# KMASAHIRO/AVR

Measured on AMD Instinct MI355X. Metric: ray-samples/sec/GPU (1024 rays×256 samp×512 freq) + IR render ms/pose, higher is better.
Workload: dtype f32; 1 GPU; c2_meshrir_1024x256x512; mode=pose, rays=1024, samples=256, T=1022, freq_bins=512, distinct_poses=16, parallelism=poses x1 (no data-path collective)

## Files before the change

avr_amd/csrc/render_fwd.hip:

```cpp
#include "common.h"

#include <cstdlib>

using namespace avr;

typedef float floatx16 __attribute__((ext_vector_type(16)));

namespace {

constexpr double kTwoPi = 6.283185307179586476925286766559;

__global__ void tables_kernel(avr_render_params p, float* __restrict__ d_vals,
                              float* __restrict__ frac, int32_t* __restrict__ shift,
                              float* __restrict__ pl, float2* __restrict__ phase,
                              float2* __restrict__ tw) {
    const int S = p.n_samples, T = p.T, F = T / 2 + 1;
    const int64_t gid = (int64_t)blockIdx.x * blockDim.x + threadIdx.x;
    const int64_t stride = (int64_t)gridDim.x * blockDim.x;
    for (int64_t i = gid; i < S; i += stride) {
        const float d = linspace_at(0.0f, 1.0f, S, (int)i) * p.depth_scale + p.depth_offset;
        const float fr = (p.fs * d) / p.speed;
        d_vals[i] = d;
        frac[i] = fr;
        shift[i] = (int32_t)rintf(fr);
// ... 232 lines not shown
            const float al = alpha[s];
            alpha[s] = trans * al;
            trans = trans * ((1.0f - al) + 1e-6f);
        }
    }
    __syncthreads();
    if (active)
        for (int s = lane; s < S; s += 64) w_out[base + s] = alpha[s];
}

constexpr int kMaxReduceThreads = 1024;
constexpr int kMaxGroupRays = 4096;

template <typename Tin, bool VECTOR, int CPT, int kUnroll, int G, int MAXT>
__global__ __launch_bounds__(MAXT) void ray_reduce_fwd_kernel(
    avr_render_params pp, const Tin* __restrict__ sig, const float* __restrict__ w,
    const int32_t* __restrict__ delay, float* __restrict__ part, int B, int R, int S, int T,
    int rays_per_split, int64_t total) {
    constexpr int VEC = VECTOR ? Vec16<Tin>::N : 1;
    extern __shared__ float lds_wd[];
    const int nthreads = blockDim.x;
    const int split = blockIdx.x, s0 = blockIdx.y * G, b = blockIdx.z;
    const int gcount = min(G, S - s0);
    const int r0 = split * rays_per_split;
    const int nr = max(0, min(R, r0 + rays_per_split) - r0);
    float* w_l = lds_wd;
    int* d_l = reinterpret_cast<int*>(lds_wd + G * max(nr, 1));
    for (int i = threadIdx.x; i < G * nr; i += nthreads) {
        const int g = i / nr, rr = i - g * nr;
        if (g < gcount) {
            const int64_t idx = ((int64_t)b * R + r0 + rr) * S + s0 + g;
            w_l[i] = w[idx];
            d_l[i] = delay[idx];
        } else {
            w_l[i] = 0.0f;
            d_l[i] = 0x7fffffff;
        }
    }
    __syncthreads();
    const int64_t row0 = (((int64_t)b * R + r0) * S + s0) * (int64_t)T;
    const int L = gcount * T;
    const int phase = (int)(row0 % VEC);
    const int nchunks = (L + phase + VEC - 1) / VEC;
    const int64_t row_stride = (int64_t)S * T;

    float acc[CPT][VEC];
    int tk[CPT][VEC];
    int tm[CPT][VEC];
    int gk[CPT][VEC];
    int tmax[CPT][G];
    int lim[G];
#pragma unroll
    for (int g = 0; g < G; ++g) lim[g] = tail_limit(pp, min(s0 + g, S - 1));
#pragma unroll
    for (int c = 0; c < CPT; ++c) {
#pragma unroll
        for (int g = 0; g < G; ++g) tmax[c][g] = -1;
#pragma unroll
        for (int k = 0; k < VEC; ++k) {
            acc[c][k] = 0.0f;
            const int e = (threadIdx.x + c * nthreads) * VEC + k - phase;
            const bool ok = e >= 0 && e < L;
            const int g = (G == 1) ? 0 : (ok ? e / T : 0);
            gk[c][k] = g;
            tk[c][k] = ok ? e - g * T : -1;
            int l = lim[0];
#pragma unroll
            for (int q = 1; q < G; ++q)
                if (g == q) l = lim[q];
            tm[c][k] = (tk[c][k] >= 0 && tk[c][k] < l) ? tk[c][k] : -1;
#pragma unroll
            for (int q = 0; q < G; ++q)
                if (g == q) tmax[c][q] = max(tmax[c][q], tm[c][k]);
        }
    }

    auto live = [&](int r, int c) {
        bool any = false;
#pragma unroll
        for (int g = 0; g < G; ++g) any |= tmax[c][g] >= d_l[g * nr + r];
        return any;
    };
    auto load_chunk = [&](int64_t rowbase, int c, bool need, float* x) {
        const int j = threadIdx.x + c * nthreads;
        if constexpr (VECTOR) {
            load16_masked(sig + rowbase, (uint32_t)nchunks * 16u,
                          need ? (uint32_t)j * 16u : kSkip, x);
        } else {
            const int64_t e0 = rowbase + j;
            x[0] = (need && j < nchunks && e0 < total) ? load_f(sig, e0) : 0.0f;
        }
    };
    auto accumulate = [&](int r, float (*x)[VEC]) {
        float wg[G];
        int dg[G];
#pragma unroll
        for (int g = 0; g < G; ++g) {
            wg[g] = w_l[g * nr + r];
            dg[g] = d_l[g * nr + r];
        }
#pragma unroll
        for (int c = 0; c < CPT; ++c)
#pragma unroll
            for (int k = 0; k < VEC; ++k) {
                float ws = wg[0];
                int ds = dg[0];
#pragma unroll
                for (int g = 1; g < G; ++g)
                    if (gk[c][k] == g) {
                        ws = wg[g];
                        ds = dg[g];
                    }
                const float wm = (tm[c][k] >= ds) ? ws : 0.0f;
                acc[c][k] = fmaf(wm, x[c][k], acc[c][k]);
            }
    };

    int r = 0;
    for (; r + kUnroll <= nr; r += kUnroll) {
        float x[kUnroll][CPT][VEC];
        bool need[kUnroll][CPT];
#pragma unroll
        for (int u = 0; u < kUnroll; ++u)
#pragma unroll
            for (int c = 0; c < CPT; ++c) need[u][c] = live(r + u, c);
#pragma unroll
        for (int u = 0; u < kUnroll; ++u) {
            const int64_t rowbase = row0 + (int64_t)(r + u) * row_stride - phase;
#pragma unroll
            for (int c = 0; c < CPT; ++c) load_chunk(rowbase, c, need[u][c], x[u][c]);
        }
#pragma unroll
        for (int u = 0; u < kUnroll; ++u) accumulate(r + u, x[u]);
    }
    for (; r < nr; ++r) {
        const int64_t rowbase = row0 + (int64_t)r * row_stride - phase;
        float x[CPT][VEC];
#pragma unroll
        for (int c = 0; c < CPT; ++c) load_chunk(rowbase, c, live(r, c), x[c]);
        accumulate(r, x);
    }
#pragma unroll
    for (int c = 0; c < CPT; ++c)
#pragma unroll
        for (int k = 0; k < VEC; ++k) {
            const int t = tk[c][k];
            if (t >= 0) part[(((int64_t)split * B + b) * S + s0 + gk[c][k]) * T + t] = acc[c][k];
        }
}

constexpr int kDftThreads = 256;
constexpr int kKc = 64;

template <int NS>
__global__ __launch_bounds__(kDftThreads) void dft_phase_fwd_kernel(
    avr_render_params pp, const float* __restrict__ part, const float* __restrict__ pl,
    const int32_t* __restrict__ shift, const float2* __restrict__ phase,
    const float2* __restrict__ twg, float2* __restrict__ spart, int B, int S, int T, int KS,
    int kchunk, int xcd_order) {
    extern __shared__ float2 tw[];
    __shared__ float As[32][kKc + 1];
    const int F = T / 2 + 1;
    const int P = ((S + 31) / 32) * KS;
    (void)P;
    const int nfb = (F + 127) / 128, nst = (S + 31) / 32;
    const int per = KS * nfb;
    int stile, q;
    if (xcd_order) {
        const int L = blockIdx.x, xcd = L & 7;
        q = L >> 3;
        stile = (q / per) * 8 + xcd;
        if (stile >= nst) return;
    } else {
        stile = blockIdx.x / per;
        q = blockIdx.x;
    }
    const int ks = (q % per) / nfb, fblk = (q % per) % nfb;
    const int b = blockIdx.z;
    const int wave = threadIdx.x >> 6, lane = threadIdx.x & 63;
    const int fbase = fblk * 128 + wave * 32;
    const int f = fbase + (lane & 31);
    const int fm = (f < F) ? f : 0;
    const int half = lane >> 5;
    const int col = threadIdx.x & 63, row0 = threadIdx.x >> 6;
    int sh[8];
    bool srow[8];
#pragma unroll
    for (int i = 0; i < 8; ++i) {
        const int s = stile * 32 + row0 + 4 * i;
        srow[i] = s < S;
        sh[i] = receiver_shift(pp, min(s, S - 1));
    }
    (void)shift;
    const int64_t slab = (int64_t)B * S * T;
    const int s_first = min(stile * 32 + row0, S - 1);
    const int64_t rowbase0 = ((int64_t)b * S + s_first) * T;
    const int64_t max_row_off = ((int64_t)b * S + (S - 1)) * T;

    const int k0 = ks * kchunk;
    const int k1 = min(T, k0 + kchunk);
    floatx16 acc_re, acc_im;
#pragma unroll
    for (int i = 0; i < 16; ++i) {
        acc_re[i] = 0.0f;
        acc_im[i] = 0.0f;
    }
    const int inc = (int)((2LL * fm) % T);
    float raw[NS][8], g[8];
    auto issue = [&](int kc) {
        const int tc = min(kc + col, T - 1);
#pragma unroll
        for (int k = 0; k < NS; ++k)
#pragma unroll
            for (int i = 0; i < 8; ++i) {
                const int64_t ro = min(rowbase0 + (int64_t)(4 * i) * T, max_row_off);
                raw[k][i] = part[k * slab + ro + tc];
            }
#pragma unroll
        for (int i = 0; i < 8; ++i) g[i] = pl[sh[i] + tc];
    };
    auto commit = [&](int kc) {
        const int t = kc + col;
#pragma unroll
        for (int i = 0; i < 8; ++i) {
            float sum = raw[0][i];
#pragma unroll
            for (int k = 1; k < NS; ++k) sum += raw[k][i];
            const bool ok = srow[i] && t < k1 && t < T - 1 - sh[i];
            As[row0 + 4 * i][col] = ok ? sum * g[i] : 0.0f;
        }
    };
    if (k0 < k1) issue(k0);
    stage_table<kDftThreads>(tw, twg, T);
    for (int kc = k0; kc < k1; kc += kKc) {
        __syncthreads();
        commit(kc);
        __syncthreads();
        if (kc + kKc < k1) issue(kc + kKc);
        int idx = (int)(((int64_t)(kc + half) * fm) % T);
#pragma unroll 8
        for (int kk = 0; kk < kKc; kk += 2) {
            const float a = As[lane & 31][kk + half];
            float2 c = tw[idx];
            asm volatile("" : "+v"(c.x), "+v"(c.y));
            acc_re = __builtin_amdgcn_mfma_f32_32x32x2f32(a, c.x, acc_re, 0, 0, 0);
            acc_im = __builtin_amdgcn_mfma_f32_32x32x2f32(a, c.y, acc_im, 0, 0, 0);
            idx += inc;
            if (idx >= T) idx -= T;
        }
    }
    float re = 0.0f, im = 0.0f;
    {
        float2 ph[16];
#pragma unroll
        for (int reg = 0; reg < 16; ++reg) {
            const int s = stile * 32 + (reg & 3) + 8 * (reg >> 2) + 4 * half;
            ph[reg] = phase[(int64_t)min(s, S - 1) * F + fm];
        }
#pragma unroll
        for (int reg = 0; reg < 16; ++reg) asm volatile("" ::"v"(ph[reg].x), "v"(ph[reg].y));
#pragma unroll
        for (int reg = 0; reg < 16; ++reg) {
            const int s = stile * 32 + (reg & 3) + 8 * (reg >> 2) + 4 * half;
            if (s < S) {
                const float zr = acc_re[reg], zi = acc_im[reg];
                re += zr * ph[reg].x - zi * ph[reg].y;
                im += zr * ph[reg].y + zi * ph[reg].x;
            }
        }
    }
    re += __shfl_xor(re, 32, 64);
    im += __shfl_xor(im, 32, 64);
    if (half == 0 && f < F) {
        spart[((int64_t)b * P + stile * KS + ks) * F + f] = make_float2(re, im);
    }
}

__global__ __launch_bounds__(256) void spectrum_finalize_kernel(int B, int P, int F,
                                                                const float2* __restrict__ spart,
                                                                float2* __restrict__ out) {
    __shared__ float2 red[16][17];
    const int b = blockIdx.y;
    const int g = threadIdx.x >> 4, j = threadIdx.x & 15;
    const int f = blockIdx.x * 16 + j;
    const int fc = min(f, F - 1);
    const float2* src = spart + (int64_t)b * P * F + fc;
    float ax = 0.f, ay = 0.f;
    for (int q0 = 0; q0 < P; q0 += 64) {
        float2 v[4];
#pragma unroll
        for (int u = 0; u < 4; ++u) v[u] = src[(int64_t)min(q0 + g + 16 * u, P - 1) * F];
#pragma unroll
        for (int u = 0; u < 4; ++u)
            if (q0 + g + 16 * u < P) {
                ax += v[u].x;
                ay += v[u].y;
            }
    }
    red[g][j] = make_float2(ax, ay);
    __syncthreads();
    if (g == 0 && f < F) {
        float2 r = red[0][j];
        for (int k = 1; k < 16; ++k) {
            r.x += red[k][j].x;
            r.y += red[k][j].y;
        }
        out[(int64_t)b * F + f] = r;
    }
}

__global__ __launch_bounds__(256) void irfft_kernel(int F, int B1, const float2* __restrict__ spec,
                                                    const float2* __restrict__ spec2,
                                                    const float2* __restrict__ twg,
                                                    float* __restrict__ ir, float* __restrict__ ir2) {
    extern __shared__ float2 lds[];
    __shared__ float red[8][33];
    const int n = 2 * (F - 1);
    float2* X = lds;
    float2* tw = lds + F;
    int b = blockIdx.y;
    if (b >= B1) {
        b -= B1;
        spec = spec2;
        ir = ir2;
    }
    stage_table<256>(X, spec + (int64_t)b * F, F);
    stage_table<256>(tw, twg, n);
    __syncthreads();
    const int tl = threadIdx.x & 31, slice = threadIdx.x >> 5;
    const int t = blockIdx.x * 32 + tl;
    const int tm = (t < n) ? t : 0;
    float acc[4] = {0.f, 0.f, 0.f, 0.f};
    int idx[4];
#pragma unroll
    for (int c = 0; c < 4; ++c) idx[c] = (int)(((int64_t)(1 + slice + 8 * c) * tm) % n);
    const int step4 = (int)((32LL * tm) % n);
    int k = 1 + slice;
    for (; k + 24 < F - 1; k += 32) {
#pragma unroll
        for (int c = 0; c < 4; ++c) {
            const float2 w = tw[idx[c]];
            const float2 x = X[k + 8 * c];
            acc[c] += x.x * w.x - x.y * w.y;
            idx[c] += step4;
            if (idx[c] >= n) idx[c] -= n;
        }
    }
    for (; k < F - 1; k += 8) {
        const int id = (int)(((int64_t)k * tm) % n);
        const float2 w = tw[id];
        const float2 x = X[k];
        acc[0] += x.x * w.x - x.y * w.y;
    }
    red[slice][tl] = (acc[0] + acc[1]) + (acc[2] + acc[3]);
    __syncthreads();
    if (slice == 0 && t < n) {
        float s = 0.0f;
#pragma unroll
        for (int q = 0; q < 8; ++q) s += red[q][tl];
        const float nyq = (t & 1) ? -X[F - 1].x : X[F - 1].x;
        const float v = (X[0].x + nyq) + 2.0f * s;
        ir[(int64_t)b * n + t] = v / (float)n;
    }
}

__global__ __launch_bounds__(256) void irfft_bwd_kernel(int F, const float* __restrict__ gir,
                                                        const float2* __restrict__ twg,
                                                        float2* __restrict__ grad) {
    extern __shared__ float lds_irb[];
    __shared__ float2 red[8][33];
    const int n = 2 * (F - 1);
    const int b = blockIdx.y;
    float2* tw = reinterpret_cast<float2*>(lds_irb);
    float* g = lds_irb + 2 * n;
    stage_table<256>(tw, twg, n);
    for (int i = threadIdx.x; i < n; i += 256) g[i] = gir[(int64_t)b * n + i];
    __syncthreads();
    const int kl = threadIdx.x & 31, sl = threadIdx.x >> 5;
    const int k = blockIdx.x * 32 + kl;
    const int km = k < F ? k : 0;
    int idx = (int)(((int64_t)km * sl) % n);
    const int step = (int)(((int64_t)km * 8) % n);
    float ac = 0.f, as = 0.f;
    for (int t = sl; t < n; t += 8) {
        const float2 c = tw[idx];
        ac = fmaf(g[t], c.x, ac);
        as = fmaf(g[t], c.y, as);
        idx += step;
        if (idx >= n) idx -= n;
    }
    red[sl][kl] = make_float2(ac, as);
    __syncthreads();
    if (sl == 0 && k < F) {
        float2 r = red[0][kl];
        for (int q = 1; q < 8; ++q) {
            r.x += red[q][kl].x;
            r.y += red[q][kl].y;
        }
        const bool edge = (k == 0) || (k == F - 1);
// ... 153 lines not shown
        (void)hipFuncSetAttribute((const void*)weights_fwd_kernel<__hip_bfloat16>,
                                  hipFuncAttributeMaxDynamicSharedMemorySize, (int)lds);
    }
    if (attn_dtype == AVR_DTYPE_F32)
        hipLaunchKernelGGL(weights_fwd_kernel<float>, grid, dim3(256), lds, as_stream(stream), *p,
                           (int)B, (const float*)attn, rays_o, pos_tx, dirs, d_vals, w, delay);
    else if (attn_dtype == AVR_DTYPE_F16)
        hipLaunchKernelGGL(weights_fwd_kernel<__half>, grid, dim3(256), lds, as_stream(stream),
                           *p, (int)B, (const __half*)attn, rays_o, pos_tx, dirs, d_vals, w, delay);
    else if (attn_dtype == AVR_DTYPE_BF16)
        hipLaunchKernelGGL(weights_fwd_kernel<__hip_bfloat16>, grid, dim3(256), lds,
                           as_stream(stream), *p, (int)B, (const __hip_bfloat16*)attn, rays_o,
                           pos_tx, dirs, d_vals, w, delay);
    else
        return fail(AVR_E_ARG, "avr_weights_fwd: unknown attn dtype");
    return check_launch("avr_weights_fwd");
}


namespace {
int reduce_variant() { return 2; }

struct ReduceShape {
    int G, cpt, threads;
};

template <int VEC>
ReduceShape reduce_shape(int S, int T) {
    ReduceShape sh;
    sh.G = 1;
    int max_phase = 0;
    for (int s0 = 0; s0 < S && s0 < VEC * sh.G; s0 += sh.G)
        max_phase = max(max_phase, (int)(((int64_t)s0 * T) % VEC));
    const int nch = (sh.G * T + max_phase + VEC - 1) / VEC;
    sh.cpt = 1;
    while ((nch + sh.cpt - 1) / sh.cpt > kMaxReduceThreads) ++sh.cpt;
    const int need = (nch + sh.cpt - 1) / sh.cpt;
    sh.threads = max(64, (need + 63) / 64 * 64);
    return sh;
}

template <typename Tin, bool VECTOR, int C, int G>
void launch_reduce_v(dim3 grid, dim3 block, size_t lds, hipStream_t st, const avr_render_params& pp,
                     const Tin* s, const float* w,
                     const int32_t* delay, float* part, int B, int R, int S, int T, int rps,
                     int64_t total) {
    const bool u8 = reduce_variant() == 3;
    if (block.x <= 512) {
        if (u8)
            hipLaunchKernelGGL((ray_reduce_fwd_kernel<Tin, VECTOR, C, 8, G, 512>), grid, block,
                               lds, st, pp, s, w, delay, part, B, R, S, T, rps, total);
        else
            hipLaunchKernelGGL((ray_reduce_fwd_kernel<Tin, VECTOR, C, 4, G, 512>), grid, block,
                               lds, st, pp, s, w, delay, part, B, R, S, T, rps, total);
    } else {
        if (u8)
            hipLaunchKernelGGL((ray_reduce_fwd_kernel<Tin, VECTOR, C, 8, G, 1024>), grid, block,
                               lds, st, pp, s, w, delay, part, B, R, S, T, rps, total);
        else
            hipLaunchKernelGGL((ray_reduce_fwd_kernel<Tin, VECTOR, C, 4, G, 1024>), grid, block,
                               lds, st, pp, s, w, delay, part, B, R, S, T, rps, total);
    }
}

template <typename Tin, bool VECTOR>
int launch_reduce(const avr_render_params* p, int B, const void* sig, const float* w,
                  const int32_t* delay, int n_split, float* part, hipStream_t st) {
    constexpr int VEC = VECTOR ? Vec16<Tin>::N : 1;
    const int R = n_rays(*p), S = p->n_samples, T = p->T;
    const int rps = (R + n_split - 1) / n_split;
    const ReduceShape sh = reduce_shape<VEC>(S, T);
    if (sh.G * rps > kMaxGroupRays)
        return fail(AVR_E_ARG, "avr_ray_reduce_fwd: too many rays per split (raise n_split)");
    const int64_t total = (int64_t)B * R * S * T;
    const dim3 grid(n_split, (S + sh.G - 1) / sh.G, B);
    const dim3 block(sh.threads);
    const size_t lds = (size_t)sh.G * max(rps, 1) * 8;
    const Tin* s = (const Tin*)sig;
#define AVR_RR(C, GG)                                                                              \
    if (sh.cpt == C && sh.G == GG)                                                                 \
        return launch_reduce_v<Tin, VECTOR, C, GG>(grid, block, lds, st, *p, s, w, delay, part, B, R, S, \
                                                   T, rps, total),                                 \
               check_launch("avr_ray_reduce_fwd");
    AVR_RR(1, 1) AVR_RR(1, 2) AVR_RR(1, 4) AVR_RR(2, 1) AVR_RR(2, 2) AVR_RR(2, 4) AVR_RR(3, 1)
    AVR_RR(4, 1)
#undef AVR_RR
    return fail(AVR_E_CONFIG, "ray_reduce: T too long for this build");
}
}

extern "C" int avr_reduce_splits(const avr_render_params* p, int32_t B, int32_t sig_dtype,
                                 int32_t* n_split) {
    if (int e = validate(p)) return e;
    AVR_REQUIRE(B >= 1 && n_split, "avr_reduce_splits: bad args");
    const int R = n_rays(*p), S = p->n_samples, T = p->T;
    const int vec = (sig_dtype == AVR_DTYPE_F16 || sig_dtype == AVR_DTYPE_BF16) ? 8 : 4;
    const ReduceShape sh = vec == 8 ? reduce_shape<8>(S, T) : reduce_shape<4>(S, T);
    const int groups = (S + sh.G - 1) / sh.G;
    auto rps = [&](int k) { return (R + k - 1) / k; };
    if (const char* f = getenv("AVR_NSPLIT")) {
        const int v = atoi(f);
        if ((v == 1 || v == 2 || v == 4 || v == 8 || v == 16) && v <= R && rps(v) * sh.G <= kMaxGroupRays) {
            *n_split = v;
            return 0;
        }
    }
    const int64_t waves_target = (vec == 8) ? 4096 : 1536;
    const int64_t waves_per_split = (int64_t)groups * B * (sh.threads / 64);
    int n = 1;
    while (n < 16 && (n * waves_per_split < waves_target || rps(n) * sh.G > kMaxGroupRays) &&
           rps(2 * n) >= 8)
        n *= 2;
    if (rps(n) * sh.G > kMaxGroupRays) return fail(AVR_E_CONFIG, "avr_reduce_splits: too many rays");
    *n_split = n;
    return 0;
}

extern "C" int avr_ray_reduce_fwd(const avr_render_params* p, int32_t B, const void* signal,
                                  int32_t sig_dtype, const float* w, const int32_t* delay,
                                  int32_t n_split, float* part, void* stream) {
    if (int e = validate(p)) return e;
    AVR_REQUIRE(B >= 1 && signal && w && delay && part, "avr_ray_reduce_fwd: null pointer");
    const int R = n_rays(*p);
    AVR_REQUIRE(n_split >= 1 && n_split <= R, "avr_ray_reduce_fwd: n_split out of range");
    AVR_REQUIRE((R + n_split - 1) / n_split <= kMaxGroupRays,
                "avr_ray_reduce_fwd: too many rays per split (raise n_split)");
    const int64_t st = (int64_t)p->n_samples * p->T;
    const bool aligned = (reinterpret_cast<uintptr_t>(signal) % 16) == 0;
    hipStream_t s = as_stream(stream);
    if (sig_dtype == AVR_DTYPE_F32) {
        if (aligned && st % 4 == 0) return launch_reduce<float, true>(p, B, signal, w, delay, n_split, part, s);
        return launch_reduce<float, false>(p, B, signal, w, delay, n_split, part, s);
    }
    if (sig_dtype == AVR_DTYPE_F16) {
        if (aligned && st % 8 == 0) return launch_reduce<__half, true>(p, B, signal, w, delay, n_split, part, s);
        return launch_reduce<__half, false>(p, B, signal, w, delay, n_split, part, s);
    }
    if (sig_dtype == AVR_DTYPE_BF16) {
        if (aligned && st % 8 == 0)
            return launch_reduce<__hip_bfloat16, true>(p, B, signal, w, delay, n_split, part, s);
        return launch_reduce<__hip_bfloat16, false>(p, B, signal, w, delay, n_split, part, s);
    }
    return fail(AVR_E_ARG, "avr_ray_reduce_fwd: unknown signal dtype");
}

extern "C" int avr_dft_phase_fwd(const avr_render_params* p, int32_t B, const float* part,
                                 int32_t n_split, const float* pl_table, const int32_t* shift,
                                 const float* phase, const float* twiddle, int32_t k_split,
                                 float* spart, void* stream) {
    if (int e = validate(p)) return e;
    AVR_REQUIRE(B >= 1 && part && pl_table && shift && phase && twiddle && spart,
                "avr_dft_phase_fwd: null pointer");
    const int S = p->n_samples, T = p->T, F = T / 2 + 1;
    const int nkc = (T + kKc - 1) / kKc;
    AVR_REQUIRE(k_split >= 1 && k_split <= nkc, "avr_dft_phase_fwd: k_split out of range");
    const int kchunk = ((nkc + k_split - 1) / k_split) * kKc;
    const int nst = (S + 31) / 32;
    const int xcd_order = nst >= 8;
    const int per = k_split * ((F + 127) / 128);
    const dim3 grid((unsigned)(xcd_order ? 8 * ((nst + 7) / 8) * per : nst * per), 1, B);
    const size_t lds = (size_t)T * sizeof(float2);
    auto go = [&](auto kern) {
        if (lds > 65536)
            (void)hipFuncSetAttribute((const void*)kern, hipFuncAttributeMaxDynamicSharedMemorySize,
                                      (int)lds);
        hipLaunchKernelGGL(kern, grid, dim3(kDftThreads), lds, as_stream(stream), *p, part, pl_table,
                           shift, reinterpret_cast<const float2*>(phase),
                           reinterpret_cast<const float2*>(twiddle),
                           reinterpret_cast<float2*>(spart), (int)B, S, T, (int)k_split, kchunk, xcd_order);
    };
    switch (n_split) {
        case 1: go(dft_phase_fwd_kernel<1>); break;
        case 2: go(dft_phase_fwd_kernel<2>); break;
        case 4: go(dft_phase_fwd_kernel<4>); break;
        case 8: go(dft_phase_fwd_kernel<8>); break;
        case 16: go(dft_phase_fwd_kernel<16>); break;
        default: return fail(AVR_E_ARG, "avr_dft_phase_fwd: n_split must be 1, 2, 4, 8 or 16");
    }
    return check_launch("avr_dft_phase_fwd");
}

extern "C" int avr_spectrum_finalize(int32_t B, int32_t P, int32_t F, const float* spart,
                                     float* out, void* stream) {
    AVR_REQUIRE(B >= 1 && P >= 1 && F >= 1 && spart && out, "avr_spectrum_finalize: bad args");
    hipLaunchKernelGGL(spectrum_finalize_kernel, dim3((unsigned)((F + 15) / 16), B), dim3(256), 0,
                       as_stream(stream), (int)B, (int)P, (int)F,
                       reinterpret_cast<const float2*>(spart), reinterpret_cast<float2*>(out));
    return check_launch("avr_spectrum_finalize");
}

namespace avr {
int launch_irfft(int B, int F, const float* spec, const float* spec2, const float* tw, float* ir,
                 float* ir2, void* stream) {
    AVR_REQUIRE(B >= 1 && F >= 2 && spec && tw && ir, "avr_irfft: bad args");
    const int n = 2 * (F - 1);
    AVR_REQUIRE(n <= 16384, "avr_irfft: n too large");
    const size_t lds = (size_t)(F + n) * sizeof(float2);
    const int rows = spec2 ? 2 * B : B;
    hipLaunchKernelGGL(irfft_kernel, dim3((n + 31) / 32, rows), dim3(256), lds, as_stream(stream),
                       (int)F, (int)B, reinterpret_cast<const float2*>(spec),
                       reinterpret_cast<const float2*>(spec2 ? spec2 : spec),
                       reinterpret_cast<const float2*>(tw), ir, ir2 ? ir2 : ir);
    return check_launch("avr_irfft");
}
}

extern "C" int avr_irfft(int32_t B, int32_t F, const float* spec, const float* tw, float* ir,
                         void* stream) {
    return avr::launch_irfft(B, F, spec, nullptr, tw, ir, nullptr, stream);
}

extern "C" int avr_irfft_bwd(int32_t B, int32_t F, const float* grad_ir, const float* tw,
                             float* grad_spec, void* stream) {
    AVR_REQUIRE(B >= 1 && F >= 2 && grad_ir && tw && grad_spec, "avr_irfft_bwd: bad args");
    const int n = 2 * (F - 1);
    const size_t lds = (size_t)n * (sizeof(float2) + sizeof(float));
    AVR_REQUIRE(lds <= 160 * 1024, "avr_irfft_bwd: n too large for LDS");
    if (lds > 65536)
        (void)hipFuncSetAttribute((const void*)irfft_bwd_kernel, hipFuncAttributeMaxDynamicSharedMemorySize,
                                  (int)lds);
    hipLaunchKernelGGL(irfft_bwd_kernel, dim3((F + 31) / 32, B), dim3(256), lds, as_stream(stream), (int)F,
                       grad_ir, reinterpret_cast<const float2*>(tw), reinterpret_cast<float2*>(grad_spec));
    return check_launch("avr_irfft_bwd");
}

namespace {
struct CoreLayout {
    int64_t w, delay, part, spart, bytes;
    int32_t n_split, k_split, P;
};

CoreLayout core_layout(const avr_render_params* p, int B, int sig_dtype) {
    CoreLayout L{};
    const int64_t R = n_rays(*p), S = p->n_samples, T = p->T, F = T / 2 + 1;
    int32_t ns = 1;
    avr_reduce_splits(p, B, sig_dtype, &ns);
    L.n_split = ns;
    const int nkc = (int)((T + kKc - 1) / kKc);
    int ks = 1;
    if (const char* f = getenv("AVR_KSPLIT")) {
        ks = atoi(f);
    } else {
        const int64_t base = ((F + 127) / 128) * ((S + 31) / 32) * B;
        ks = (int)((256 + (base > 0 ? base : 1) - 1) / (base > 0 ? base : 1));
    }
    if (ks < 1) ks = 1;
    if (ks > nkc) ks = nkc;
    L.k_split = ks;
    L.P = (int32_t)(((S + 31) / 32) * ks);
    auto al = [](int64_t x) { return (x + 255) & ~(int64_t)255; };
    int64_t o = 0;
    L.w = o;
    o += al((int64_t)B * R * S * 4);
    L.delay = o;
    o += al((int64_t)B * R * S * 4);
    L.part = o;
    o += al((int64_t)ns * B * S * T * 4);
    L.spart = o;
    o += al((int64_t)B * L.P * F * 8);
    L.bytes = o;
    return L;
}
}

extern "C" int avr_render_core_layout(const avr_render_params* p, int32_t B, int32_t sig_dtype,
                                      int64_t* offsets ,
                                      int32_t* splits ) {
    if (int e = validate(p)) return e;
    AVR_REQUIRE(B >= 1 && offsets && splits, "avr_render_core_layout: bad args");
    const CoreLayout L = core_layout(p, B, sig_dtype);
    offsets[0] = L.w;
    offsets[1] = L.delay;
    offsets[2] = L.part;
    offsets[3] = L.spart;
    offsets[4] = L.bytes;
    splits[0] = L.n_split;
    splits[1] = L.k_split;
    return 0;
}

extern "C" int avr_render_core_fwd(const avr_render_params* p, int32_t B, const void* attn,
                                   int32_t attn_dtype, const void* signal, int32_t sig_dtype,
                                   const float* rays_o, const float* pos_tx, const float* dirs,
                                   const avr_table_ptrs* tab, void* workspace,
                                   int64_t workspace_bytes, float* out, float* ir, void* ev_begin,
                                   void* ev_end, void* stream) {
    if (int e = validate(p)) return e;
    AVR_REQUIRE(tab && workspace && out, "avr_render_core_fwd: null pointer");
    const CoreLayout L = core_layout(p, B, sig_dtype);
    AVR_REQUIRE(workspace_bytes >= L.bytes, "avr_render_core_fwd: workspace too small");
    char* ws = reinterpret_cast<char*>(workspace);
    float* w = reinterpret_cast<float*>(ws + L.w);
    int32_t* delay = reinterpret_cast<int32_t*>(ws + L.delay);
    float* part = reinterpret_cast<float*>(ws + L.part);
    float* spart = reinterpret_cast<float*>(ws + L.spart);
    if (int e = avr_weights_fwd(p, B, attn, attn_dtype, rays_o, pos_tx, dirs, tab->d_vals, w, delay, stream))
        return e;
    hipStream_t s = as_stream(stream);
    if (ev_begin) (void)hipEventRecord(reinterpret_cast<hipEvent_t>(ev_begin), s);
    if (int e = avr_ray_reduce_fwd(p, B, signal, sig_dtype, w, delay, L.n_split, part, stream))
        return e;
    if (ev_end) (void)hipEventRecord(reinterpret_cast<hipEvent_t>(ev_end), s);
    if (int e = avr_dft_phase_fwd(p, B, part, L.n_split, tab->pl_table, tab->shift, tab->phase, tab->twiddle,
                                  L.k_split, spart, stream))
        return e;
    if (int e = avr_spectrum_finalize(B, L.P, p->T / 2 + 1, spart, out, stream)) return e;
    if (ir) {
        AVR_REQUIRE(tab->ir_twiddle, "avr_render_core_fwd: ir requested without ir_twiddle");
        return avr_irfft(B, p->T / 2 + 1, out, tab->ir_twiddle, ir, stream);
    }
    return 0;
}
```

avr_amd/renderer.py:

```python
from __future__ import annotations

import ctypes
import math
import threading

import torch
import torch.nn as nn

from . import _lib
from ._lib import DTYPE_BF16, DTYPE_F16, DTYPE_F32, render_params
from .options import tuning_env
from .wcache import cache_lookup, cache_store, capturing, cast_weight


_RENDER_KEYS = ("n_samples", "near", "far", "n_azi", "n_ele", "speed", "fs", "pathloss",
                "xyz_min", "xyz_max")


def _ptr(t):
    return None if t is None else t.data_ptr()


def _stream(device):
    return torch.cuda.current_stream(device).cuda_stream


class _NoGuard:
    def __enter__(self):
        return None

    def __exit__(self, *exc):
        return False


_NO_GUARD = _NoGuard()


def _on(dev):
    return _NO_GUARD if torch.cuda.current_device() == dev.index else torch.cuda.device(dev)


def _f32_on(t, dev):
    if t.device != dev or t.dtype != torch.float32:
        t = t.to(dev, torch.float32)
    return t if t.is_contiguous() else t.contiguous()


def _dtype_code(t):
    if t.dtype == torch.float32:
        return DTYPE_F32
    if t.dtype == torch.float16:
        return DTYPE_F16
    if t.dtype == torch.bfloat16:
        return DTYPE_BF16
    raise TypeError(f"unsupported dtype {t.dtype} (float32, float16 or bfloat16)")


class Tables:

    def __init__(self, p, device):
        S, T = p.n_samples, p.T
        F = T // 2 + 1
        f32 = dict(dtype=torch.float32, device=device)
        self.d_vals = torch.empty(S, **f32)
        self.frac = torch.empty(S, **f32)
        self.shift = torch.empty(S, dtype=torch.int32, device=device)
        self.pl = torch.empty(p.pl_len, **f32)
        self.phase = torch.empty(S, F, 2, **f32)
        self.twiddle = torch.empty(T, 2, **f32)
        n = 2 * (F - 1)
        self.ir_n = n
        self.ir_twiddle = torch.empty(max(n, 2), 2, **f32)
        st = _stream(device)
        with torch.cuda.device(device):
            _lib.call("avr_tables", ctypes_ref(p), _ptr(self.d_vals), _ptr(self.frac),
                      _ptr(self.shift), _ptr(self.pl), _ptr(self.phase), _ptr(self.twiddle), st)
            if n >= 2:
                _lib.call("avr_ir_twiddle", n, _ptr(self.ir_twiddle), st)
        shifts = self.shift.cpu()
        self.max_shift = int(shifts.max().item()) if S > 0 else 0
        self.ptrs = _lib.TablePtrs(self.d_vals.data_ptr(), self.shift.data_ptr(),
                                   self.pl.data_ptr(), self.phase.data_ptr(),
                                   self.twiddle.data_ptr(),
                                   self.ir_twiddle.data_ptr() if n >= 2 else None)
        self._layouts = {}

    def core_layout(self, p, B, sig_code):
        key = (p.n_rays, B, sig_code) + tuning_env()
        v = self._layouts.get(key)
        if v is None:
            with _TABLE_LOCK:
                v = self._layouts.get(key)
                if v is None:
                    off = (ctypes.c_int64 * 5)()
                    sp = (ctypes.c_int32 * 2)()
                    _lib.call("avr_render_core_layout", ctypes_ref(p), B, sig_code, off, sp)
                    v = (tuple(off), int(sp[0]), int(sp[1]))
                    self._layouts[key] = v
        return v


def ctypes_ref(p):
    import ctypes

    return ctypes.byref(p)


_TABLE_CACHE: dict = {}
_TABLE_LOCK = threading.RLock()


def get_tables(p, device) -> Tables:
    key = (device.index, p.key())
    t = _TABLE_CACHE.get(key)
    if t is None:
        with _TABLE_LOCK:
            t = _TABLE_CACHE.get(key)
            if t is None:
                t = Tables(p, device)
                _TABLE_CACHE[key] = t
    return t


def check_config(p, tables: Tables):
    if p.near_clamp + 1 >= p.pl_len:
        raise IndexError("path_loss[prev_part+1] out of range (renderer.py:99): "
                         f"int(0.1/speed*fs)+1 = {p.near_clamp + 1} >= {p.pl_len}")
    if tables.max_shift + p.T > p.pl_len:
        raise RuntimeError(
            "stack expects each tensor to be equal size: receiver delay "
            f"{tables.max_shift} samples + T={p.T} exceeds the path-loss table ({p.pl_len}); "
            "the reference fails the same way at renderer.py:100 (needs shift <= 1.5T)")


def reduce_splits(p, B, sig_code):
    import ctypes

    n = ctypes.c_int32(0)
    _lib.call("avr_reduce_splits", ctypes_ref(p), B, sig_code, ctypes.byref(n))
    return int(n.value)


def pick_k_split(B, S, T):
    F = T // 2 + 1
    nkc = math.ceil(T / 64)
    forced = tuning_env()[1]
    forced = int(forced) if forced else None
    if forced:
        return max(1, min(nkc, forced))
    base = math.ceil(F / 128) * math.ceil(S / 32) * B
    return max(1, min(nkc, math.ceil(256 / max(1, base))))


def _weights(p, attn, rays_o, position_tx, dirs, tables, st):
    B = attn.size(0)
    R, S = p.n_rays, p.n_samples
    dev = attn.device
    w = torch.empty(B, R, S, dtype=torch.float32, device=dev)
    delay = torch.empty(B, R, S, dtype=torch.int32, device=dev)
    _lib.call("avr_weights_fwd", ctypes_ref(p), B, _ptr(attn), _dtype_code(attn), _ptr(rays_o),
              _ptr(position_tx), _ptr(dirs), _ptr(tables.d_vals), _ptr(w), _ptr(delay), st)
    return w, delay


def _spectrum(p, tables, part, n_split, B, dev, st):
    S, T = p.n_samples, p.T
    F = T // 2 + 1
    k_split = pick_k_split(B, S, T)
    P = math.ceil(S / 32) * k_split
    spart = torch.empty(B, P, F, 2, dtype=torch.float32, device=dev)
    _lib.call("avr_dft_phase_fwd", ctypes_ref(p), B, _ptr(part), n_split, _ptr(tables.pl),
              _ptr(tables.shift), _ptr(tables.phase), _ptr(tables.twiddle), k_split,
              _ptr(spart), st)
    out = torch.empty(B, F, 2, dtype=torch.float32, device=dev)
    _lib.call("avr_spectrum_finalize", B, P, F, _ptr(spart), _ptr(out), st)
    return out


def _grad_z(p, tables, grad_out, B, dev, st):
    g = grad_out.contiguous().float()
    gz = torch.empty(B, p.n_samples, p.T, dtype=torch.float32, device=dev)
    _lib.call("avr_dft_phase_bwd", ctypes_ref(p), B, _ptr(g), _ptr(tables.pl), _ptr(tables.shift),
              _ptr(tables.phase), _ptr(tables.twiddle), _ptr(gz), st)
    return gz


def _grad_attn(p, tables, attn, grad_w, st):
    grad_attn = torch.empty_like(attn)
    _lib.call("avr_weights_bwd", ctypes_ref(p), attn.size(0), _ptr(attn), _dtype_code(attn),
              _ptr(tables.d_vals), _ptr(grad_w), _ptr(grad_attn), st)
    return grad_attn


def _render_core_fwd(attn, signal, p, tables, rays_o, position_tx, dirs, ir_out, timer=None):
    dev = signal.device
    B = signal.size(0)
    F = p.T // 2 + 1
    sig_code = _dtype_code(signal)
    off, n_split, _ = tables.core_layout(p, B, sig_code)
    ws = torch.empty(off[4], dtype=torch.uint8, device=dev)
    out = torch.empty(B, F, 2, dtype=torch.float32, device=dev)
    ev0 = ev1 = None
    if timer is not None:
        R, S = p.n_rays, p.n_samples
        delay = ws[off[1]:off[1] + B * R * S * 4].view(torch.int32).view(B, R, S)
        ev0, ev1 = timer.events(n_split=n_split, delay=delay, shift=tables.shift)
    _lib.call("avr_render_core_fwd", ctypes_ref(p), B, _ptr(attn), _dtype_code(attn),
              _ptr(signal), sig_code, _ptr(rays_o), _ptr(position_tx), _ptr(dirs),
              ctypes.byref(tables.ptrs), _ptr(ws), off[4], _ptr(out), _ptr(ir_out), ev0, ev1,
              _stream(dev))
    return out, ws, off


class RenderCore(torch.autograd.Function):

    @staticmethod
    def forward(ctx, attn, signal, p, tables, rays_o, position_tx, dirs, ir_out=None, timer=None):
        out, ws, off = _render_core_fwd(attn, signal, p, tables, rays_o, position_tx, dirs, ir_out, timer)
        B, R, S = signal.size(0), p.n_rays, p.n_samples
        w = ws[off[0]:off[0] + B * R * S * 4].view(torch.float32).view(B, R, S)
        delay = ws[off[1]:off[1] + B * R * S * 4].view(torch.int32).view(B, R, S)
        ctx.p, ctx.tables = p, tables
        ctx.save_for_backward(attn, signal, w, delay)
        return out

    @staticmethod
    def backward(ctx, grad_out):
        attn, signal, w, delay = ctx.saved_tensors
        p, tables = ctx.p, ctx.tables
        dev = signal.device
        B = signal.size(0)
        R, S = p.n_rays, p.n_samples
        st = _stream(dev)
        gz = _grad_z(p, tables, grad_out, B, dev, st)
        grad_signal = torch.empty_like(signal)
        grad_w = torch.empty(B, R, S, dtype=torch.float32, device=dev)
        _lib.call("avr_ray_reduce_bwd", ctypes_ref(p), B, _ptr(signal), _dtype_code(signal),
                  _ptr(gz), _ptr(w), _ptr(delay), _ptr(grad_signal), _ptr(grad_w), st)
        grad_attn = _grad_attn(p, tables, attn, grad_w, st) if ctx.needs_input_grad[0] else None
        return (grad_attn, grad_signal if ctx.needs_input_grad[1] else None,
                None, None, None, None, None, None, None)


def _packed_head_weight(w_master, W, cache, pref, shape_key, st):
    key = (W.data_ptr(), w_master._version, shape_key)
    cache = cache and not capturing()
    if cache:
        hit = cache_lookup(w_master, "_avr_headpack", key)
        if hit is not None:
            return hit
    B, K, code = shape_key[2], shape_key[3], shape_key[4]
    Wp = torch.empty_like(W)
    _lib.call("avr_head_pack_w", pref, B, K, _ptr(W), code, _ptr(Wp), st)
    return cache_store(w_master, "_avr_headpack", key, Wp) if cache else Wp


def _packed_exact_weight(w_master, W, cache, pref, shape_key, nbytes, st):
    key = (W.data_ptr(), w_master._version, shape_key)
    cache = cache and not capturing()
    if cache:
        hit = cache_lookup(w_master, "_avr_exactpack", key)
        if hit is not None:
            return hit
    K, code = shape_key[1], shape_key[2]
    Wf = torch.empty(nbytes // 2, dtype=W.dtype, device=W.device)
    _lib.call("avr_head_pack_w_exact", pref, K, _ptr(W), code, _ptr(Wf), st)
    return cache_store(w_master, "_avr_exactpack", key, Wf) if cache else Wf


class FusedHeadCore(torch.autograd.Function):

    @staticmethod
    def forward(ctx, attn, h, w_master, dtype, p, tables, rays_o, position_tx, dirs, cache=False, exact=False,
                relu_h=False, timer=None):
        dev = h.device
        B, K = h.size(0), h.size(-1)
        S, T = p.n_samples, p.T
        st = _stream(dev)
        pref = ctypes_ref(p)
        W = cast_weight(w_master, dtype, cache)
        code = _dtype_code(h)
        w, delay = _weights(p, attn, rays_o, position_tx, dirs, tables, st)
        R = p.n_rays
        perm = torch.empty(B, S, R, dtype=torch.int32, device=dev)
        ws = torch.empty(B, S, R, dtype=torch.float32, device=dev)
        cnt = torch.empty(B, S, T, dtype=torch.int32, device=dev)
        _lib.call("avr_head_sort", pref, B, _ptr(w), _ptr(delay), _ptr(perm), _ptr(ws), _ptr(cnt), st)
        if exact:
            ns, wbytes = ctypes.c_int32(0), ctypes.c_int64(0)
            _lib.call("avr_head_exact_layout", pref, B, K, code, ctypes.byref(ns), ctypes.byref(wbytes))
            n_split = ns.value
            part = torch.empty(n_split, B, S, T, dtype=torch.float32, device=dev)
            queue = torch.empty(256, dtype=torch.int32, device=dev)
            Wf = _packed_exact_weight(w_master, W, cache, pref, (p.T, K, code), wbytes.value, st)
            ev0, ev1 = timer.head_events(delay, tables.shift, K) if timer is not None else (None, None)
            if ev0 is not None:
                ev0.record()
            _lib.call("avr_head_fwd_exact", pref, B, K, _ptr(h), _ptr(Wf), code, _ptr(perm), _ptr(ws), _ptr(cnt),
                      _ptr(delay), n_split, _ptr(part), _ptr(queue), st)
            if ev1 is not None:
                ev1.record()
        else:
            ns = ctypes.c_int32(0)
            _lib.call("avr_head_splits", pref, B, K, code, ctypes.byref(ns))
# ... 356 lines not shown
```

Baseline: 2.305 billion ray-samples/s.

## Fold real DFT input symmetry to halve time-axis work in phase DFT

The DFT kernel now exploits cos/sin symmetry of a real input: it loads samples at t and T-t, forms their sum and difference, and runs the K loop only over F rather than T. This roughly halves the MFMA reduction length and the LDS staging passes, at the cost of twice the global loads per tile plus extra register pressure. Split partial sums are accumulated in held groups to limit live registers. The k-split heuristic is also changed to target more workgroups, using the new shorter tile count in both the host C++ and the Python picker.

After: 2.313 billion ray-samples/s, median of 6. About the same (+0.4%).

```diff
diff --git a/avr_amd/csrc/render_fwd.hip b/avr_amd/csrc/render_fwd.hip
--- a/avr_amd/csrc/render_fwd.hip
+++ b/avr_amd/csrc/render_fwd.hip
@@ -408,6 +408,13 @@
 constexpr int kDftThreads = 256;
 constexpr int kKc = 64;
 
+__host__ __device__ inline int dft_fold_tiles(int T) { return (T / 2 + 1 + kKc - 1) / kKc; }
+constexpr int kDftFillWorkgroups = 768;
+constexpr int kDftFillTiles = 8;
+
+template <int NS>
+constexpr int kDftHeld = NS > 4 ? 4 : NS;
+
 template <int NS>
 __global__ __launch_bounds__(kDftThreads) void dft_phase_fwd_kernel(
     avr_render_params pp, const float* __restrict__ part, const float* __restrict__ pl,
@@ -415,7 +422,7 @@
     const float2* __restrict__ twg, float2* __restrict__ spart, int B, int S, int T, int KS,
     int kchunk, int xcd_order) {
     extern __shared__ float2 tw[];
-    __shared__ float As[32][kKc + 1];
+    __shared__ float2 PQ[32][kKc + 1];
     const int F = T / 2 + 1;
     const int P = ((S + 31) / 32) * KS;
     (void)P;
@@ -449,12 +456,16 @@
     }
     (void)shift;
     const int64_t slab = (int64_t)B * S * T;
-    const int s_first = min(stile * 32 + row0, S - 1);
-    const int64_t rowbase0 = ((int64_t)b * S + s_first) * T;
-    const int64_t max_row_off = ((int64_t)b * S + (S - 1)) * T;
+    const char* const pb = reinterpret_cast<const char*>(part + (int64_t)b * S * T);
+    uint32_t rowoff[8];
+#pragma unroll
+    for (int i = 0; i < 8; ++i) rowoff[i] = (uint32_t)min(stile * 32 + row0 + 4 * i, S - 1) * (uint32_t)T * 4u;
+    auto ld = [&](int k, int i, uint32_t tbytes) {
+        return *reinterpret_cast<const float*>(pb + (int64_t)k * slab * 4 + (uint32_t)(rowoff[i] + tbytes));
+    };
 
     const int k0 = ks * kchunk;
-    const int k1 = min(T, k0 + kchunk);
+    const int k1 = min(F, k0 + kchunk);
     floatx16 acc_re, acc_im;
 #pragma unroll
     for (int i = 0; i < 16; ++i) {
@@ -462,28 +473,72 @@
         acc_im[i] = 0.0f;
     }
     const int inc = (int)((2LL * fm) % T);
-    float raw[NS][8], g[8];
+    constexpr int NH = kDftHeld<NS>;
+    float ra[NH][8], rb[NH][8], sa[8], sb[8], ga[8], gb[8];
     auto issue = [&](int kc) {
-        const int tc = min(kc + col, T - 1);
-#pragma unroll
-        for (int k = 0; k < NS; ++k)
+        const int tc = min(kc + col, F - 1);
+        const int tmc = min(T - tc, T - 1);
+        const uint32_t ta = (uint32_t)tc * 4u, tb = (uint32_t)tmc * 4u;
+        if constexpr (NS > NH) {
+#pragma unroll
+            for (int i = 0; i < 8; ++i) sa[i] = sb[i] = 0.0f;
+#pragma unroll
+            for (int k = 0; k < NS - NH; k += NH) {
+                float xa[NH][8], xb[NH][8];
+#pragma unroll
+                for (int j = 0; j < NH; ++j)
+#pragma unroll
+                    for (int i = 0; i < 8; ++i) {
+                        xa[j][i] = ld(k + j, i, ta);
+                        xb[j][i] = ld(k + j, i, tb);
+                    }
+#pragma unroll
+                for (int j = 0; j < NH; ++j)
+#pragma unroll
+                    for (int i = 0; i < 8; ++i) {
+                        sa[i] += xa[j][i];
+                        sb[i] += xb[j][i];
+                    }
+#pragma unroll
+                for (int i = 0; i < 8; ++i) asm volatile("" : "+v"(sa[i]), "+v"(sb[i]));
+                __builtin_amdgcn_sched_barrier(0);
+            }
+        }
+#pragma unroll
+        for (int k = 0; k < NH; ++k)
 #pragma unroll
             for (int i = 0; i < 8; ++i) {
-                const int64_t ro = min(rowbase0 + (int64_t)(4 * i) * T, max_row_off);
-                raw[k][i] = part[k * slab + ro + tc];
+                ra[k][i] = ld(NS - NH + k, i, ta);
+                rb[k][i] = ld(NS - NH + k, i, tb);
             }
 #pragma unroll
-        for (int i = 0; i < 8; ++i) g[i] = pl[sh[i] + tc];
+        for (int i = 0; i < 8; ++i) {
+            ga[i] = pl[sh[i] + tc];
+            gb[i] = pl[sh[i] + tmc];
+        }
     };
     auto commit = [&](int kc) {
-        const int t = kc + col;
+        const int t = kc + col, tm = T - t;
+        const bool in = t < k1, mir = in && t >= 1 && t < tm;
 #pragma unroll
         for (int i = 0; i < 8; ++i) {
-            float sum = raw[0][i];
-#pragma unroll
-            for (int k = 1; k < NS; ++k) sum += raw[k][i];
-            const bool ok = srow[i] && t < k1 && t < T - 1 - sh[i];
-            As[row0 + 4 * i][col] = ok ? sum * g[i] : 0.0f;
+            float xa, xb;
+            if constexpr (NS > NH) {
+                xa = sa[i] + ra[0][i];
+                xb = sb[i] + rb[0][i];
+            } else {
+                xa = ra[0][i];
+                xb = rb[0][i];
+            }
+#pragma unroll
+            for (int k = 1; k < NH; ++k) {
+                xa += ra[k][i];
+                xb += rb[k][i];
+            }
+            const int live = T - 1 - sh[i];
+            const float za = (srow[i] && in && t < live) ? xa * ga[i] : 0.0f;
+            const float zb = (srow[i] && mir && tm < live) ? xb * gb[i] : 0.0f;
+            PQ[row0 + 4 * i][col] = make_float2(za + zb, mir ? za - zb : (t == 0 ? za : 0.0f));
         }
     };
     if (k0 < k1) issue(k0);
@@ -496,11 +551,11 @@
         int idx = (int)(((int64_t)(kc + half) * fm) % T);
 #pragma unroll 8
         for (int kk = 0; kk < kKc; kk += 2) {
-            const float a = As[lane & 31][kk + half];
+            const float2 a = PQ[lane & 31][kk + half];
             float2 c = tw[idx];
             asm volatile("" : "+v"(c.x), "+v"(c.y));
-            acc_re = __builtin_amdgcn_mfma_f32_32x32x2f32(a, c.x, acc_re, 0, 0, 0);
-            acc_im = __builtin_amdgcn_mfma_f32_32x32x2f32(a, c.y, acc_im, 0, 0, 0);
+            acc_re = __builtin_amdgcn_mfma_f32_32x32x2f32(a.x, c.x, acc_re, 0, 0, 0);
+            acc_im = __builtin_amdgcn_mfma_f32_32x32x2f32(a.y, c.y, acc_im, 0, 0, 0);
             idx += inc;
             if (idx >= T) idx -= T;
         }
@@ -960,7 +1015,7 @@
     AVR_REQUIRE(B >= 1 && part && pl_table && shift && phase && twiddle && spart,
                 "avr_dft_phase_fwd: null pointer");
     const int S = p->n_samples, T = p->T, F = T / 2 + 1;
-    const int nkc = (T + kKc - 1) / kKc;
+    const int nkc = dft_fold_tiles(T);
     AVR_REQUIRE(k_split >= 1 && k_split <= nkc, "avr_dft_phase_fwd: k_split out of range");
     const int kchunk = ((nkc + k_split - 1) / k_split) * kKc;
     const int nst = (S + 31) / 32;
@@ -1044,13 +1099,15 @@
     int32_t ns = 1;
     avr_reduce_splits(p, B, sig_dtype, &ns);
     L.n_split = ns;
-    const int nkc = (int)((T + kKc - 1) / kKc);
+    const int nkc = dft_fold_tiles((int)T);
     int ks = 1;
     if (const char* f = getenv("AVR_KSPLIT")) {
         ks = atoi(f);
     } else {
-        const int64_t base = ((F + 127) / 128) * ((S + 31) / 32) * B;
-        ks = (int)((256 + (base > 0 ? base : 1) - 1) / (base > 0 ? base : 1));
+        const int64_t base = std::max<int64_t>(1, ((F + 127) / 128) * ((S + 31) / 32) * B);
+        ks = (int)((256 + base - 1) / base);
+        const int fill = (int)std::min<int64_t>((kDftFillWorkgroups + base - 1) / base, nkc / kDftFillTiles);
+        if (fill > ks) ks = fill;
     }
     if (ks < 1) ks = 1;
     if (ks > nkc) ks = nkc;
diff --git a/avr_amd/renderer.py b/avr_amd/renderer.py
--- a/avr_amd/renderer.py
+++ b/avr_amd/renderer.py
@@ -143,13 +143,14 @@
 
 def pick_k_split(B, S, T):
     F = T // 2 + 1
-    nkc = math.ceil(T / 64)
+    nkc = math.ceil(F / 64)
     forced = tuning_env()[1]
     forced = int(forced) if forced else None
     if forced:
         return max(1, min(nkc, forced))
-    base = math.ceil(F / 128) * math.ceil(S / 32) * B
-    return max(1, min(nkc, math.ceil(256 / max(1, base))))
+    base = max(1, math.ceil(F / 128) * math.ceil(S / 32) * B)
+    ks = max(math.ceil(256 / base), min(math.ceil(768 / base), nkc // 8))
+    return max(1, min(nkc, ks))
 
 
 def _weights(p, attn, rays_o, position_tx, dirs, tables, st):
```
